# jondo2010/rust-ida

Hardware: AMD Instinct MI355X
Metric: Newton iters/sec (fp64), batched dense DAE N=512 B=4096 (higher is better)
Workload: dtype f64; 1 GPU; random linear dense index-1 DAE F=A y'+B y-c (SURVEY 8(d) config 3), N=512, B=4096 systems per GPU, rtol 1e-6 atol 1e-8, t=0..1 with 10 outputs, every system restarts on its own when it reaches t=1 (endless stream of integrations); n=512, batch_per_gpu=4096, total_batch=4096, lu_period=1, groups_per_gpu=4, mutually_concurrent_streams=4

## Files before the change

### rust-ida_amd/csrc/exp_switches.hpp

```cpp
#pragma once

#if !defined(IDAHIP_TIMING_BUILD) &&                                                                                   \
    (defined(IDAHIP_EXP_NOPRO) || defined(IDAHIP_EXP_NOUPD) || defined(IDAHIP_EXP_NOGATHER) || defined(IDAHIP_EXP_NODIAG) || \
     defined(IDAHIP_EXP_NOSWEEP) || defined(IDAHIP_STAMPS) || defined(IDAHIP_TRAIL_PIPE) || defined(IDAHIP_TRAIL_QUAD) ||   \
     defined(IDAHIP_WP_RING) || defined(IDAHIP_US_PAD) || defined(IDAHIP_SYS_UNR) || defined(IDAHIP_TRAIL_AHEAD) ||         \
     defined(IDAHIP_NT_SYS) || defined(IDAHIP_NT_SOLVE) || defined(IDAHIP_NT_FINALIZE) || defined(IDAHIP_NT_TRAIL))
#error "IDAHIP_EXP_* / IDAHIP_STAMPS / IDAHIP_TRAIL_* (IDAHIP_TRAIL_AHEAD: 0..3) / IDAHIP_WP_RING / IDAHIP_US_PAD / IDAHIP_SYS_UNR / IDAHIP_NT_* are timing-build switches: add -DIDAHIP_TIMING_BUILD (the library then reports itself as one and is not a product)"
#endif

namespace idahip {
namespace tb {

#ifdef IDAHIP_TIMING_BUILD
constexpr bool TIMING_BUILD = true;
#else
constexpr bool TIMING_BUILD = false;
#endif

#ifdef IDAHIP_EXP_NOPRO
constexpr bool NOPRO = true;
#else
constexpr bool NOPRO = false;
#endif
#ifdef IDAHIP_EXP_NOUPD
constexpr bool NOUPD = true;
#else
constexpr bool NOUPD = false;
#endif
#ifdef IDAHIP_EXP_NOGATHER
constexpr bool NOGATHER = true;
#else
constexpr bool NOGATHER = false;
#endif
#ifdef IDAHIP_EXP_NODIAG
constexpr bool NODIAG = true;
#else
constexpr bool NODIAG = false;
#endif
#ifdef IDAHIP_EXP_NOSWEEP
constexpr bool NOSWEEP = true;
#else
constexpr bool NOSWEEP = false;
#endif
#ifdef IDAHIP_STAMPS
constexpr int STAMPS = IDAHIP_STAMPS;
#else
constexpr int STAMPS = -1;
#endif
#ifdef IDAHIP_TRAIL_PIPE
constexpr bool TRAIL_PIPE = IDAHIP_TRAIL_PIPE != 0;
#else
constexpr bool TRAIL_PIPE = true;
#endif
#ifdef IDAHIP_TRAIL_QUAD
constexpr bool TRAIL_QUAD = IDAHIP_TRAIL_QUAD != 0;
#else
constexpr bool TRAIL_QUAD = true;
#endif
#ifdef IDAHIP_US_PAD
constexpr int US_PAD = IDAHIP_US_PAD;
#else
constexpr int US_PAD = 2;
#endif
#ifdef IDAHIP_TRAIL_AHEAD
constexpr int trail_ahead(int kk) { return IDAHIP_TRAIL_AHEAD; }
#else
constexpr int trail_ahead(int kk) { return kk < 32 ? 1 : 3; }
#endif
#ifdef IDAHIP_WP_RING
constexpr bool WP_DEEP_RING = IDAHIP_WP_RING != 0;
#else
constexpr bool WP_DEEP_RING = false;
#endif
#ifdef IDAHIP_SYS_UNR
constexpr int SYS_UNR = IDAHIP_SYS_UNR;
#else
constexpr int SYS_UNR = 16;
#endif

#ifdef IDAHIP_NT_SYS
constexpr bool NT_SYS = IDAHIP_NT_SYS != 0;
#else
constexpr bool NT_SYS = true;
#endif
#ifdef IDAHIP_NT_SOLVE
constexpr bool NT_SOLVE = IDAHIP_NT_SOLVE != 0;
#else
constexpr bool NT_SOLVE = true;
#endif
#ifdef IDAHIP_NT_FINALIZE
constexpr bool NT_FINALIZE = IDAHIP_NT_FINALIZE != 0;
#else
constexpr bool NT_FINALIZE = true;
#endif
#ifdef IDAHIP_NT_TRAIL
constexpr bool NT_TRAIL = IDAHIP_NT_TRAIL != 0;
#else
constexpr bool NT_TRAIL = false;
#endif

}
}
```

### rust-ida_amd/csrc/idahip.hip

```cpp
#include "common.hpp"
#include "lu_kernels.hpp"
#include "lu_driver.hpp"
#include "problem_kernels.hpp"
#include "solve_kernels.hpp"
#include "band_kernels.hpp"
#include "dq_kernels.hpp"
#include "vector_kernels.hpp"
#include "ic_kernels.hpp"
#include "tiny_ida.hpp"
#include "round_ida.hpp"

using namespace idahip;

namespace {

template <class T>
int dalloc(idahip_ctx* c, T** p, size_t count) {
    *p = nullptr;
    if (count == 0) return 0;
    IDAHIP_HIP(c, hipMalloc((void**)p, count * sizeof(T)));
    return 0;
}

int check_list(idahip_ctx* c, const int32_t* hIdx, int nsys) {
// ... 1819 lines not shown
        if (e == hipSuccess) e = hipStreamSynchronize(c->stream);
        if (e != hipSuccess) rc = fail(c, -100, "idahip_pow_batch: %s", hipGetErrorString(e));
    }
    if (dx) (void)hipFree(dx);
    if (dy) (void)hipFree(dy);
    if (dout) (void)hipFree(dout);
    return rc;
}

static int stepper_buffers(idahip_ctx* c, const idahip_tiny_call* call, bool outputs);

static FlowArgs flow_args(idahip_ctx* c, const idahip_tiny_call* call) {
    FlowArgs f;
    f.touts = c->tiny_touts; f.ntout = call->ntout; f.recycle = call->recycle; f.resume = call->resume;
    f.mxstep = call->mxstep; f.maxord = call->maxord; f.maxnef = call->maxnef; f.maxncf = call->maxncf;
    f.epcon = call->epcon; f.hmax_inv = call->hmax_inv; f.t0 = call->t0;
    f.start_round = call->start_round ? (const long long*)c->tiny_start : nullptr;
    f.acc = (unsigned long long*)c->tiny_acc;
    f.batch = c->batch;
    f.nrt = call->nroots;
    for (int i = 0; i < call->nroots && i < IDAHIP_MAX_ROOTS; ++i) {
        f.rt_comp[i] = call->root_comps[i];
        f.rt_thr[i] = call->root_thresholds[i];
    }
    return f;
}

int idahip_tiny_solve(idahip_ctx* c, void* hSys, size_t sys_bytes, const idahip_tiny_call* call, int64_t* hRoundsDone, uint64_t* hAcc,
                      double* hYout, double* hYPout) {
    DevGuard dev_guard__(c);
    if (!c) return -1;
    if (!hSys || !call || !hRoundsDone || !hAcc || !call->touts || call->ntout < 1) return fail(c, -2, "null argument");
    if (sys_bytes != sizeof(idactl::SysCore)) return fail(c, -2, "controller state of %zu bytes, this library expects %zu", sys_bytes, sizeof(idactl::SysCore));
    if (c->n != 3 || (c->kind != IDAHIP_ROBERTS && c->kind != IDAHIP_LORENZ63))
        return fail(c, -2, "the device-resident stepper takes the Roberts and Lorenz63 problems (n = 3)");
    if (c->jac_dq && !c->h_constr.empty()) return fail(c, -2, "difference-quotient Jacobians and constraints do not combine (DESIGN.md section 4g)");
    if (call->recycle && (!c->ic_y || !c->ic_yp)) return fail(c, -2, "recycle needs idahip_snapshot_initial");
    if (call->recycle && call->max_rounds < 1) return fail(c, -2, "recycle needs a round limit");
    const int batch = c->batch, n = c->n;
    int rc = stepper_buffers(c, call, hYout || hYPout);
    if (rc) return rc;
    const size_t ysz = (size_t)call->ntout * batch * n;
    IDAHIP_HIP(c, hipMemcpyAsync(c->tiny_sys, hSys, (size_t)batch * sizeof(idactl::SysCore), hipMemcpyHostToDevice, c->stream));
    IDAHIP_HIP(c, hipMemcpyAsync(c->tiny_touts, call->touts, sizeof(double) * call->ntout, hipMemcpyHostToDevice, c->stream));
    if (call->start_round)
        IDAHIP_HIP(c, hipMemcpyAsync(c->tiny_start, call->start_round, sizeof(int64_t) * batch, hipMemcpyHostToDevice, c->stream));
    IDAHIP_HIP(c, hipMemsetAsync(c->tiny_acc, 0, 2 * sizeof(uint64_t), c->stream));
    TinyIdaArgs a;
    a.sys = (idactl::SysCore*)c->tiny_sys;
    a.v = vec_state(c);
    a.savres = c->savres; a.lu = c->lu; a.piv = (long long*)c->piv; a.params = c->params; a.nparam = c->nparam;
    a.ic_y = c->ic_y; a.ic_yp = c->ic_yp;
    a.f = flow_args(c, call);
    a.roots = (idahip_root_state*)c->tiny_roots;
    a.jac_dq = c->jac_dq;
    a.max_rounds = call->max_rounds;
    a.round_base = call->round_base;
    a.yout = hYout ? c->tiny_yout : nullptr;
    a.ypout = hYPout ? c->tiny_ypout : nullptr;
    a.rounds_done = (long long*)c->tiny_rounds;
    {
        KTimer kt(c, IDAHIP_K_VECTOR, batch);
        int spw = 64;
        {
            const int simds = c->simds > 0 ? c->simds : 1024;
            while (spw > 1 && (long)(batch + spw / 2 - 1) / (spw / 2) <= simds / 4) spw >>= 1;
            if (const char* e = std::getenv("IDAHIP_TINY_SPW")) {
                const int v = (int)std::strtol(e, nullptr, 10);
                if (v == 1 || v == 2 || v == 4 || v == 8 || v == 16 || v == 32 || v == 64) spw = v;
            }
        }
        const size_t lds_state = (size_t)spw * sizeof(idactl::SysCore), lds_all = lds_state + (size_t)spw * sizeof(double) * tiny_lds_doubles(n);
        const bool roots = call->nroots > 0;
        const bool constr = !c->h_constr.empty();
        auto kern = c->kind == IDAHIP_ROBERTS ? (roots ? tiny_ida_kernel<IDAHIP_ROBERTS, true, false> : tiny_ida_kernel<IDAHIP_ROBERTS, false, false>)
                                              : (roots ? tiny_ida_kernel<IDAHIP_LORENZ63, true, false> : tiny_ida_kernel<IDAHIP_LORENZ63, false, false>);
        if (constr)
            kern = c->kind == IDAHIP_ROBERTS ? (roots ? tiny_ida_kernel<IDAHIP_ROBERTS, true, true> : tiny_ida_kernel<IDAHIP_ROBERTS, false, true>)
                                             : (roots ? tiny_ida_kernel<IDAHIP_LORENZ63, true, true> : tiny_ida_kernel<IDAHIP_LORENZ63, false, true>);
        const int lds_vec = hipFuncSetAttribute((const void*)kern, hipFuncAttributeMaxDynamicSharedMemorySize, (int)(64 * (sizeof(idactl::SysCore) + sizeof(double) * tiny_lds_doubles(n)))) == hipSuccess ? 1 : 0;
        if (!lds_vec) (void)hipGetLastError();
        const size_t shm = lds_vec ? lds_all : lds_state;
        hipLaunchKernelGGL(kern, dim3((batch + spw - 1) / spw), dim3(spw), shm, c->stream, a, lds_vec, constr ? (const double*)c->d_constr : (const double*)nullptr);
        if ((rc = post_launch(c, "tiny_ida"))) return rc;
    }
    IDAHIP_HIP(c, hipMemcpyAsync(hSys, c->tiny_sys, (size_t)batch * sizeof(idactl::SysCore), hipMemcpyDeviceToHost, c->stream));
    if (call->nroots > 0)
        IDAHIP_HIP(c, hipMemcpyAsync(call->root_states, c->tiny_roots, (size_t)batch * sizeof(idahip_root_state), hipMemcpyDeviceToHost, c->stream));
    IDAHIP_HIP(c, hipMemcpyAsync(hRoundsDone, c->tiny_rounds, sizeof(int64_t) * batch, hipMemcpyDeviceToHost, c->stream));
    IDAHIP_HIP(c, hipMemcpyAsync(hAcc, c->tiny_acc, 2 * sizeof(uint64_t), hipMemcpyDeviceToHost, c->stream));
    if (hYout) IDAHIP_HIP(c, hipMemcpyAsync(hYout, c->tiny_yout, sizeof(double) * ysz, hipMemcpyDeviceToHost, c->stream));
    if (hYPout) IDAHIP_HIP(c, hipMemcpyAsync(hYPout, c->tiny_ypout, sizeof(double) * ysz, hipMemcpyDeviceToHost, c->stream));
    IDAHIP_HIP(c, hipStreamSynchronize(c->stream));
    return 0;
}

static int stepper_buffers(idahip_ctx* c, const idahip_tiny_call* call, bool outputs) {
    const int batch = c->batch, n = c->n;
    int rc = 0;
    if (!c->tiny_sys) IDAHIP_HIP(c, hipMalloc(&c->tiny_sys, (size_t)batch * sizeof(idactl::SysCore)));
    if (!c->tiny_start) rc |= dalloc(c, &c->tiny_start, (size_t)batch);
    if (!c->tiny_rounds) rc |= dalloc(c, &c->tiny_rounds, (size_t)batch);
    if (!c->tiny_acc) rc |= dalloc(c, &c->tiny_acc, (size_t)2);
    if (rc) return rc;
    if (call->nroots < 0 || call->nroots > IDAHIP_MAX_ROOTS) return fail(c, -2, "the device steppers take at most %d root functions", IDAHIP_MAX_ROOTS);
    if (call->nroots > 0) {
        if (!call->root_comps || !call->root_thresholds || !call->root_states) return fail(c, -2, "root functions without their arrays");
        for (int i = 0; i < call->nroots; ++i)
            if (call->root_comps[i] < 0 || call->root_comps[i] >= n) return fail(c, -2, "root function %d watches component %d of %d", i, call->root_comps[i], n);
        if (call->recycle) return fail(c, -2, "root finding and idaens_stream's restarts do not combine");
        if (!c->tiny_roots) IDAHIP_HIP(c, hipMalloc(&c->tiny_roots, (size_t)batch * sizeof(idahip_root_state)));
        IDAHIP_HIP(c, hipMemcpyAsync(c->tiny_roots, call->root_states, (size_t)batch * sizeof(idahip_root_state), hipMemcpyHostToDevice, c->stream));
    }
    if (call->ntout > c->tiny_ntout_cap) {
        if (c->tiny_touts) (void)hipFree(c->tiny_touts);
        c->tiny_touts = nullptr;
        if ((rc = dalloc(c, &c->tiny_touts, (size_t)call->ntout))) return rc;
        c->tiny_ntout_cap = call->ntout;
    }
    if (outputs && call->ntout > c->tiny_yout_cap) {
        const size_t ysz = (size_t)call->ntout * batch * n;
        if (c->tiny_yout) (void)hipFree(c->tiny_yout);
        if (c->tiny_ypout) (void)hipFree(c->tiny_ypout);
        c->tiny_yout = c->tiny_ypout = nullptr;
        if ((rc = dalloc(c, &c->tiny_yout, ysz))) return rc;
        if ((rc = dalloc(c, &c->tiny_ypout, ysz))) return rc;
        c->tiny_yout_cap = call->ntout;
    }
    return 0;
}

int idahip_round_solve(idahip_ctx* c, void* hSys, size_t sys_bytes, const idahip_tiny_call* call, int64_t* hRoundsDone, uint64_t* hAcc,
                       double* hYout, double* hYPout, int64_t* rounds_run) {
    DevGuard dev_guard__(c);
    if (!c) return -1;
    if (!hSys || !call || !hRoundsDone || !hAcc || !rounds_run || !call->touts || call->ntout < 1) return fail(c, -2, "null argument");
    if (sys_bytes != sizeof(idactl::SysCore)) return fail(c, -2, "controller state of %zu bytes, this library expects %zu", sys_bytes, sizeof(idactl::SysCore));
    const bool lin = c->kind == IDAHIP_LINEAR_DENSE && c->n <= LU_BIG_MAX_N;
    const bool heat = c->kind == IDAHIP_HEAT1D && c->n <= LU_BIG_MAX_N;
    if (c->n <= TINY_N || !(lin || heat) || c->lu_variant < 4)
        return fail(c, -2, "the device-resident lock-step stepper takes linear dense and heat problems with %d < n <= %d (LU variant 4)", TINY_N, LU_BIG_MAX_N);
    if (!c->h_constr.empty()) return fail(c, -2, "the device lock-step stepper does not check constraints: the host stepper does (DESIGN.md section 4g)");
    if (call->recycle && (!c->ic_y || !c->ic_yp)) return fail(c, -2, "recycle needs idahip_snapshot_initial");
    if (call->recycle && call->max_rounds < 1) return fail(c, -2, "recycle needs a round limit");
    const int batch = c->batch, n = c->n;
    const long nn = (long)n * n;
    int rc = stepper_buffers(c, call, hYout || hYPout);
    if (rc) return rc;
    if (!c->rnd_i) rc |= dalloc(c, &c->rnd_i, (size_t)8 * batch + 8 + 2 * IDAHIP_K_COUNT);
    if (!c->rnd_d) rc |= dalloc(c, &c->rnd_d, (size_t)4 * batch);
    if (rc) return rc;
    if (!c->rnd_host) IDAHIP_HIP(c, hipHostMalloc((void**)&c->rnd_host, 4 * sizeof(int32_t)));
    const size_t ysz = (size_t)call->ntout * batch * n;
    IDAHIP_HIP(c, hipMemcpyAsync(c->tiny_sys, hSys, (size_t)batch * sizeof(idactl::SysCore), hipMemcpyHostToDevice, c->stream));
    IDAHIP_HIP(c, hipMemcpyAsync(c->tiny_touts, call->touts, sizeof(double) * call->ntout, hipMemcpyHostToDevice, c->stream));
    if (call->start_round)
        IDAHIP_HIP(c, hipMemcpyAsync(c->tiny_start, call->start_round, sizeof(int64_t) * batch, hipMemcpyHostToDevice, c->stream));
    IDAHIP_HIP(c, hipMemsetAsync(c->tiny_acc, 0, 2 * sizeof(uint64_t), c->stream));
    RoundArgs a;
    a.f = flow_args(c, call);
    a.sys = (idactl::SysCore*)c->tiny_sys;
    a.v = vec_state(c);
    a.ic_y = c->ic_y; a.ic_yp = c->ic_yp;
    a.yout = hYout ? c->tiny_yout : nullptr;
    a.ypout = hYPout ? c->tiny_ypout : nullptr;
    a.round_base = call->round_base;
    a.fused_jac = (c->kind == IDAHIP_LINEAR_DENSE && !c->jac_dq) ? 1 : 0;
    if (c->jac_dq && !c->dq_hh && (rc = dalloc(c, &c->dq_hh, (size_t)batch))) return rc;
    a.lu_period = c->lu_period;
    a.roots = (idahip_root_state*)c->tiny_roots;
    int* ib = c->rnd_i;
    a.stepping = ib; a.in_newton = ib + batch; a.skipP = ib + 2 * batch; a.skipL = ib + 3 * batch; a.skipI = ib + 4 * batch;
    a.skipS = ib + 5 * batch; a.ident = ib + 6 * batch; a.lu_list = ib + 7 * batch; a.lu_cnt = ib + 8 * batch; a.summary = ib + 8 * batch + 1; a.lu_wait = ib + 8 * batch + 3;
    a.stats = (unsigned long long*)(ib + 8 * batch + 4);
    if (((uintptr_t)a.stats & 7) != 0) a.stats = (unsigned long long*)(ib + 8 * batch + 5);
    IDAHIP_HIP(c, hipMemsetAsync(a.stats, 0, IDAHIP_K_COUNT * sizeof(unsigned long long), c->stream));
    a.lu_info = c->lu_info;
    a.tn = c->rnd_d; a.cj = c->rnd_d + batch; a.scale = c->rnd_d + 2 * batch; a.nrm_out = c->rnd_d + 3 * batch;
    a.rounds_done = (long long*)c->tiny_rounds;
    hipLaunchKernelGGL(round_init_kernel, dim3((batch + 255) / 256), dim3(256), 0, c->stream, a);
    IDAHIP_HIP(c, hipMemsetAsync(a.summary, 0, 2 * sizeof(int), c->stream));
    const size_t shm_wg = sizeof(double) * (4 * (size_t)n + 8);
    const size_t shm_it = 2 * sizeof(double) * n;
    SysArgs sa;
    fill_sys_args(c, sa, 1);
    sa.idx = a.ident; sa.tn = a.tn; sa.cj = a.cj;
    int64_t r = 0;
    for (;; ++r) {
        if (call->max_rounds > 0 && r >= call->max_rounds) break;
        a.round = r;
        a.first_round = r == 0;
        {
            KTimer kt(c, IDAHIP_K_VECTOR, 0);
            if (call->nroots > 0) hipLaunchKernelGGL(round_begin_kernel<true>, dim3(batch), dim3(WG_NT), shm_wg, c->stream, a);
            else hipLaunchKernelGGL(round_begin_kernel<false>, dim3(batch), dim3(WG_NT), shm_wg, c->stream, a);
            hipLaunchKernelGGL(round_lists_kernel, dim3(1), dim3(1024), 0, c->stream, a);
        }
        const bool lu_cnt_on_host = n > LU_MAX_N && !c->band;
        if (lu_cnt_on_host) {
            IDAHIP_HIP(c, hipMemcpyAsync(c->rnd_host + 2, a.lu_cnt, sizeof(int), hipMemcpyDeviceToHost, c->stream));
            IDAHIP_HIP(c, hipEventRecord(c->ev_cnt, c->stream));
        }
        {
            KTimer kt(c, IDAHIP_K_SYS, 0);
            sa.reset_ee = 1; sa.skip = a.skipP;
            if ((rc = launch_sys(c, sa, batch, nullptr))) return rc;
        }
        if (a.fused_jac) {
            KTimer kt(c, IDAHIP_K_SYS_JAC, 0);
            sa.skip = a.skipL;
            if ((rc = launch_sys(c, sa, batch, c->jw))) return rc;
        } else {
            {
                KTimer kt(c, IDAHIP_K_SYS, 0);
                sa.skip = a.skipL;
                if ((rc = launch_sys(c, sa, batch, nullptr))) return rc;
            }
            KTimer kt(c, IDAHIP_K_JAC, 0);
            if (c->jac_dq)
                hipLaunchKernelGGL(dq_round_prep_kernel, dim3((batch + 255) / 256), dim3(256), 0, c->stream, a.sys, (const int*)a.skipL, c->dq_hh,
                                   batch, dq_evals(c));
            if ((rc = launch_jac(c, c->jw, a.ident, a.cj, batch, nullptr, nullptr, nullptr, a.skipL, c->dq_hh))) return rc;
        }
        {
            int nlu = batch;
            const int* d_cnt = a.lu_cnt;
            if (lu_cnt_on_host) {
                IDAHIP_HIP(c, hipEventSynchronize(c->ev_cnt));
                nlu = c->rnd_host[2];
                d_cnt = nullptr;
                if (nlu < 0 || nlu > batch) return fail(c, -4, "list length %d outside 0..%d", nlu, batch);
            }
            KTimer kt(c, IDAHIP_K_LU, 0);
            if (c->band) rc = band_factor(c, c->bab, (long)c->ldab * n, c->piv, n, c->ml, c->mu, a.lu_list, nlu, d_cnt);
            else rc = lu_factor_batched(c, c->jw, nn, c->lu, nn, (long long*)c->piv, n, c->perm, a.lu_list, nlu, d_cnt);
            if (rc) return rc;
            if ((rc = post_launch(c, "lu"))) return rc;
        }
        hipLaunchKernelGGL(round_newton_ctl_kernel, dim3((batch + 255) / 256), dim3(256), 0, c->stream, a, 0);
        for (int m = 1; m <= idactl::MAXNLSIT; ++m) {
            {
                KTimer kt(c, IDAHIP_K_NEWTON_ITER, 0);
                if ((rc = launch_newton_iter(c, a.ident, a.scale, a.nrm_out, a.skipI, batch))) return rc;
            }
            hipLaunchKernelGGL(round_newton_ctl_kernel, dim3((batch + 255) / 256), dim3(256), 0, c->stream, a, m);
            if (m < idactl::MAXNLSIT) {
                KTimer kt(c, IDAHIP_K_SYS, 0);
                sa.reset_ee = 0; sa.skip = a.skipS;
                if ((rc = launch_sys(c, sa, batch, nullptr))) return rc;
            }
        }
        IDAHIP_HIP(c, hipMemsetAsync(a.summary, 0, sizeof(int), c->stream));
        {
            KTimer kt(c, IDAHIP_K_VECTOR, 0);
            if (call->nroots > 0) hipLaunchKernelGGL(round_end_kernel<true>, dim3(batch), dim3(WG_NT), shm_wg, c->stream, a);
            else hipLaunchKernelGGL(round_end_kernel<false>, dim3(batch), dim3(WG_NT), shm_wg, c->stream, a);
            if ((rc = post_launch(c, "round_end"))) return rc;
        }
        if (!call->recycle) {
            IDAHIP_HIP(c, hipMemcpyAsync(c->rnd_host, a.summary, 2 * sizeof(int), hipMemcpyDeviceToHost, c->stream));
            IDAHIP_HIP(c, hipStreamSynchronize(c->stream));
            if (c->rnd_host[0] == 0) {
                ++r;
                break;
            }
        }
    }
    (void)shm_it;
    *rounds_run = r;
    IDAHIP_HIP(c, hipMemcpyAsync(hSys, c->tiny_sys, (size_t)batch * sizeof(idactl::SysCore), hipMemcpyDeviceToHost, c->stream));
    if (call->nroots > 0)
        IDAHIP_HIP(c, hipMemcpyAsync(call->root_states, c->tiny_roots, (size_t)batch * sizeof(idahip_root_state), hipMemcpyDeviceToHost, c->stream));
    IDAHIP_HIP(c, hipMemcpyAsync(hRoundsDone, c->tiny_rounds, sizeof(int64_t) * batch, hipMemcpyDeviceToHost, c->stream));
    IDAHIP_HIP(c, hipMemcpyAsync(hAcc, c->tiny_acc, 2 * sizeof(uint64_t), hipMemcpyDeviceToHost, c->stream));
    if (hYout) IDAHIP_HIP(c, hipMemcpyAsync(hYout, c->tiny_yout, sizeof(double) * ysz, hipMemcpyDeviceToHost, c->stream));
    if (hYPout) IDAHIP_HIP(c, hipMemcpyAsync(hYPout, c->tiny_ypout, sizeof(double) * ysz, hipMemcpyDeviceToHost, c->stream));
    unsigned long long hstats[IDAHIP_K_COUNT];
    IDAHIP_HIP(c, hipMemcpyAsync(hstats, a.stats, sizeof hstats, hipMemcpyDeviceToHost, c->stream));
    IDAHIP_HIP(c, hipStreamSynchronize(c->stream));
    for (int k = 0; k < IDAHIP_K_COUNT; ++k) c->k_systems[k] += (int64_t)hstats[k];
    c->k_systems[IDAHIP_K_VECTOR] += 2 * r * (int64_t)batch;
    return 0;
}

int idahip_lu_variant(const idahip_ctx* c) { return c ? c->lu_variant : -1; }
int idahip_timing_build(void) { return tb::TIMING_BUILD ? 1 : 0; }
int idahip_set_lu_superpanel(idahip_ctx* c, int on) {
    if (!c) return -1;
    c->lu_superpanel = on != 0 ? 1 : 0;
    return 0;
}
int idahip_lu_superpanel(const idahip_ctx* c) { return c ? c->lu_superpanel : -1; }
int idahip_set_lu_period(idahip_ctx* c, int rounds) {
    if (!c || rounds < 1 || rounds > 64) return -1;
    c->lu_period = rounds;
    return 0;
}
int idahip_lu_period(const idahip_ctx* c) { return c ? c->lu_period : -1; }

int idahip_ls_type(const idahip_ctx* c) { return c ? IDAHIP_LS_DIRECT : -1; }
int idahip_ls_num_iters(const idahip_ctx* c) { return c ? 0 : -1; }
double idahip_ls_res_norm(const idahip_ctx* c) { (void)c; return 0.0; }

#ifdef IDAHIP_STAMPS
void* idahip_debug_stamps(idahip_ctx* c, size_t words) {
    if (!c) return nullptr;
    if (!c->dbg_stamps && hipMalloc((void**)&c->dbg_stamps, words * 8) != hipSuccess) return nullptr;
    (void)hipMemset(c->dbg_stamps, 0, words * 8);
    return c->dbg_stamps;
}
#endif

int idahip_set_lu_variant(idahip_ctx* c, int variant) {
    DevGuard dev_guard__(c);
    if (!c || variant < 3 || variant > 4) return -1;
    c->lu_variant = variant;
    return 0;
}

int idahip_timing_enable(idahip_ctx* c, int on) {
    DevGuard dev_guard__(c);
    if (!c) return -1;
    c->timing = on < 0 ? 0 : (on > 2 ? 2 : on);
    return 0;
}
int idahip_timing_get(idahip_ctx* c, idahip_kclass k, double* ms, int64_t* launches, int64_t* systems) {
    DevGuard dev_guard__(c);
    if (!c || k < 0 || k >= IDAHIP_K_COUNT) return -1;
    if (ms) *ms = c->k_ms[k];
    if (launches) *launches = c->k_launches[k];
    if (systems) *systems = c->k_systems[k];
    return 0;
}
int idahip_timing_reset(idahip_ctx* c) {
    DevGuard dev_guard__(c);
    if (!c) return -1;
    for (int k = 0; k < IDAHIP_K_COUNT; ++k) {
        c->k_ms[k] = 0.0;
        c->k_launches[k] = 0;
        c->k_systems[k] = 0;
    }
    return 0;
}

}
```

### rust-ida_amd/csrc/lu_driver.hpp

```cpp
#pragma once
#include "lu_kernels.hpp"
#include "lu_wavepanel.hpp"
#include "lu_superpanel.hpp"

namespace idahip {

inline int lu_factor_batched(idahip_ctx* c, double* work, long wstride, double* out, long ostride, long long* piv, long pstride,
                             int* perm, const int* d_idx, int nsys, const int* d_cnt = nullptr) {
    const int n = c->n;
    if (nsys == 0) return 0;
    if (n <= TINY_N) {
        hipLaunchKernelGGL(tiny_getrf_kernel, dim3((nsys + 63) / 64), dim3(64), 0, c->stream, work, wstride, d_idx, nsys, n, piv,
                           pstride, perm, c->lu_info);
        return 0;
    }
    if (n > LU_BIG_MAX_N) return fail(c, -3, "blocked LU supports n <= %d in this build (n = %d)", LU_BIG_MAX_N, n);
    if (d_cnt && c->lu_variant < 4) return fail(c, -3, "a device-side list length needs LU variant 4");
    LuWs w;
    w.mats = work; w.mstride = wstride; w.idx = d_idx; w.cnt = d_cnt; w.n = n;
    w.pos = c->lu_pos; w.live = c->lu_live; w.prow = c->lu_prow; w.piv = piv; w.pstride = pstride; w.info = c->lu_info; w.redo = c->lu_redo; w.nzb = c->lu_nzb; w.bz = c->lu_bz;
    w.zmap = (out == c->lu) ? c->lu_zmap : nullptr;
    w.dirty = (out == c->lu) ? c->lu_dirty : nullptr;
    w.jwzero = (w.dirty && work == c->jw && c->lu_superpanel && n > LU_MAX_N) ? c->lu_jwzero : nullptr;
    if (!w.jwzero && c->lu_jwzero && (work == c->jw || out == c->jw))
        (void)hipMemsetAsync(c->lu_jwzero, 0, (size_t)c->batch * sizeof(int), c->stream);
    w.l11 = c->lu_l11; w.stamps = c->dbg_stamps; w.out = out; w.ostride = ostride; w.l11ld = 64;
    hipLaunchKernelGGL(lu_init_kernel, dim3(nsys), dim3(256), 0, c->stream, w);
    const int nsys8 = ((nsys + 7) / 8) * 8;
    constexpr int NB = LU_NB;
    auto panel2 = [&](int k0, int lbase) {
        const int threads = (((n - k0 + 1) / 2 + 63) / 64) * 64;
        hipLaunchKernelGGL((lu_panel2_kernel<NB, 512, 2>), dim3(nsys), dim3(threads), 0, c->stream, w, k0, lbase);
    };
    for (int k0 = 0; k0 < n; k0 += 64) {
        if (n - k0 > LU_MAX_N) {
            KTimer kt(c, IDAHIP_K_LU_PANEL, nsys);
            const int cend = (k0 + 64 < n) ? k0 + 64 : n;
            if (c->lu_superpanel) {
                if (n - k0 > LU_WIDE_ROWS) {
                    const int threads = (((n - k0 + 7) / 8 + 63) / 64) * 64;
                    hipLaunchKernelGGL((lu_superpanel_kernel<8, 512, 2>), dim3(nsys), dim3(threads), 0, c->stream, w, k0);
                } else {
                    const int threads = (((n - k0 + 3) / 4 + 63) / 64) * 64;
                    hipLaunchKernelGGL((lu_superpanel_kernel<4, 512, 2>), dim3(nsys), dim3(threads), 0, c->stream, w, k0);
                }
            } else {
            auto narrow_split = [&](int kk, int nbs) {
                const int ntiles = (n - kk - nbs + 63) / 64;
                return ntiles >= 32 ? 8 : ntiles >= 16 ? 4 : ntiles >= 8 ? 2 : 1;
            };
            if (n - k0 > LU_WIDE_ROWS) {
                constexpr int NBS = 8;
                const int threads = (((n - k0 + 7) / 8 + 63) / 64) * 64;
                for (int lb = 0; lb < 64 && k0 + lb < n; lb += NBS) {
                    hipLaunchKernelGGL((lu_panelr_kernel<NBS, 8, 512, 2>), dim3(nsys), dim3(threads), 0, c->stream, w, k0 + lb, lb);
                    if (k0 + lb + NBS < cend) {
                        const int nsplit = narrow_split(k0 + lb, NBS);
                        hipLaunchKernelGGL((lu_trail_kernel<NBS, LU_BIG_MAX_N, 4>), dim3(nsys8 * nsplit), dim3(256), 0, c->stream, w, k0 + lb, nsys, 1,
                                           cend, lb * 65, nsplit);
                    }
                }
            } else {
                constexpr int NBS = 16;
                const int threads = (((n - k0 + 3) / 4 + 63) / 64) * 64;
                for (int lb = 0; lb < 64 && k0 + lb < n; lb += NBS) {
                    hipLaunchKernelGGL((lu_panelr_kernel<NBS, 4, 512, 2>), dim3(nsys), dim3(threads), 0, c->stream, w, k0 + lb, lb);
                    if (k0 + lb + NBS < cend) {
                        const int nsplit = narrow_split(k0 + lb, NBS);
                        hipLaunchKernelGGL((lu_trail_kernel<NBS, LU_BIG_MAX_N, 4>), dim3(nsys8 * nsplit), dim3(256), 0, c->stream, w, k0 + lb, nsys, 1,
                                           cend, lb * 65, nsplit);
                    }
                }
            }
            }
        } else if (c->lu_superpanel && c->lu_variant >= 4 && n > LU_MAX_N && n - k0 >= 64) {
            KTimer kt(c, IDAHIP_K_LU_PANEL, nsys);
            const int threads = (((n - k0 + 1) / 2 + 63) / 64) * 64;
            hipLaunchKernelGGL((lu_superpanel_kernel<2, 512, 2>), dim3(nsys), dim3(threads), 0, c->stream, w, k0);
        } else if (c->lu_variant >= 4 && n - k0 <= WP_MAX_ROWS) {
            KTimer kt(c, IDAHIP_K_LU_PANEL, nsys);
            const int ns = (n - k0 + 63) / 64;
#define IDAHIP_WP_LAUNCH(NSV) \
    hipLaunchKernelGGL((lu_wavepanel_kernel<false, NSV>), dim3(nsys), dim3(64), 0, c->stream, w, k0)
#define IDAHIP_WP_SWITCH()                                                                                    \
    switch (ns) {                                                                                              \
        case 1: IDAHIP_WP_LAUNCH(1); break;                                                                 \
        case 2: IDAHIP_WP_LAUNCH(2); break;                                                                 \
        case 3: IDAHIP_WP_LAUNCH(3); break;                                                                 \
        case 4: IDAHIP_WP_LAUNCH(4); break;                                                                 \
        case 5: IDAHIP_WP_LAUNCH(5); break;                                                                 \
        case 6: IDAHIP_WP_LAUNCH(6); break;                                                                 \
        case 7: IDAHIP_WP_LAUNCH(7); break;                                                                 \
        default: IDAHIP_WP_LAUNCH(8); break;                                                                \
    }
            IDAHIP_WP_SWITCH()
            hipLaunchKernelGGL((lu_wavepanel_kernel<true, 0>), dim3(nsys), dim3(64), 0, c->stream, w, k0);
#undef IDAHIP_WP_SWITCH
#undef IDAHIP_WP_LAUNCH
        } else {
            KTimer kt(c, IDAHIP_K_LU_PANEL, nsys);
            panel2(k0, 0);
            if (n - k0 > NB) {
                const int cend = (k0 + 64 < n) ? k0 + 64 : n;
                hipLaunchKernelGGL((lu_trail_kernel<NB, LU_MAX_N, 2>), dim3(nsys8), dim3(256), 0, c->stream, w, k0, nsys, 1, cend, 0, 1);
                panel2(k0 + NB, NB);
            }
        }
        const int ntrail = n - k0 - 64;
        if (ntrail > 0) {
            KTimer kt(c, IDAHIP_K_LU_TRAIL, nsys);
            const int ncb = (ntrail + 63) / 64;
            if (n > LU_MAX_N) {
                const int nstrips = (ntrail + 15) / 16;
                int nsplit = nstrips >= 64 ? 8 : nstrips >= 32 ? 4 : nstrips >= 16 ? 2 : 1;
                while (!d_cnt && nsplit > 1 && nsys * nsplit > 512) nsplit >>= 1;
                const int nbs = nsplit > 1 ? std::min(ncb, LU_SPLIT_BLOCKS) : 0;
                hipLaunchKernelGGL(lu_u12_zero_kernel, dim3(nsys8 * ncb), dim3(256), 0, c->stream, w, k0, nsys, ncb);
                hipLaunchKernelGGL(lu_trail64w_kernel<LU_BIG_MAX_N>, dim3(nsys8 * (ncb + (nsplit - 1) * nbs)), dim3(256), 0, c->stream, w, k0, nsys, ncb, nsplit);
            } else
                hipLaunchKernelGGL(lu_trail64w_kernel<LU_MAX_N>, dim3(nsys8 * ncb), dim3(256), 0, c->stream, w, k0, nsys, ncb, 1);
        }
    }
    {
        KTimer kt(c, IDAHIP_K_LU_FINALIZE, nsys);
        hipLaunchKernelGGL(lu_finalize_kernel, dim3(nsys, (n + 31) / 32), dim3(256), 0, c->stream, w, out, ostride, perm, 32, NB,
                           n > LU_MAX_N ? (c->lu_superpanel ? 64 : 8) : 0,
                           c->lu_variant >= 4 ? ((c->lu_superpanel && n > LU_MAX_N) ? LU_MAX_N : WP_MAX_ROWS) : 0);
    }
    return 0;
}

}
```

### rust-ida_amd/csrc/lu_wavepanel.hpp

```cpp
#pragma once
#include <type_traits>

#include "lu_kernels.hpp"

namespace idahip {

constexpr int WP_MAX_ROWS = 512;
constexpr int WP_RING(int ns) { return !tb::WP_DEEP_RING ? 2 : (ns >= 1 && ns <= 2) ? 8 : (ns >= 3 && ns <= 7) ? 4 : 2; }

template <bool SLOWK, int NS>
__global__ __launch_bounds__(64, SLOWK ? 1 : (NS > 0 && NS <= 3 ? 4 : 2)) void lu_wavepanel_kernel(LuWs w, const int k0) {
    constexpr int BIG = 1 << 20;
    if (w.cnt && (int)blockIdx.x >= *w.cnt) return;
    const int b = w.idx[blockIdx.x];
    if (w.info[b] != 0) return;
    const int n = w.n;
    double* __restrict__ A = w.mats + (long)b * w.mstride;
    int* __restrict__ pos = w.pos + (long)b * n;
    int* __restrict__ live = w.live + (long)b * n;
    int* __restrict__ prow = w.prow + (long)b * n;
    long long* __restrict__ piv = w.piv + (long)b * w.pstride;
    double* __restrict__ l11 = w.l11 + (long)b * L11_STRIDE;

    const __amdgpu_buffer_rsrc_t rsrc = __builtin_amdgcn_make_buffer_rsrc(A, 0, n * n * 8, 0x00020000);
    const int m = n - k0;
    const int wsp = m < 64 ? m : 64;
    const int lane = threadIdx.x;
    const int nslots = NS > 0 ? NS : (m + 63) >> 6;
    constexpr int NSC = NS > 0 ? NS : 8;

    __shared__ int ptab[64];

    int rowid[8], rpos[8], pstep[8];
    unsigned roff[8];
    static_for<0, NSC>([&](auto st) {
        constexpr int S = decltype(st)::value;
        const int li = S * 64 + lane;
        const bool has = li < m;
        rowid[S] = has ? live[li] : 0;
        rpos[S] = has ? pos[rowid[S]] : 0x7fffffff;
        pstep[S] = has ? BIG : -1;
        roff[S] = (unsigned)rowid[S] * 8u;
    });

    auto load_block = [&](double (&x)[8][8], const int b8, const int wb) {
        static_for<0, NSC>([&](auto st) {
            constexpr int S = decltype(st)::value;
            if (S < nslots) {
                const double* __restrict__ src = A + (long)(k0 + b8) * n + rowid[S];
#pragma unroll
                for (int j = 0; j < 8; ++j) x[S][j] = (j < wb) ? src[(long)j * n] : 0.0;
            } else {
#pragma unroll
                for (int j = 0; j < 8; ++j) x[S][j] = 0.0;
            }
        });
    };
    auto store_block = [&](const double (&x)[8][8], const int b8, const int wb) {
        static_for<0, NSC>([&](auto st) {
            constexpr int S = decltype(st)::value;
            if (S < nslots && pstep[S] >= 0) {
                double* __restrict__ dst = A + (long)(k0 + b8) * n + rowid[S];
#pragma unroll
                for (int j = 0; j < 8; ++j)
                    if (j < wb) dst[(long)j * n] = x[S][j];
            }
        });
    };

    auto process = [&](auto slow_tag, double (&x)[8][8], const int b8, const int wb) -> int {
        constexpr bool SLOW = decltype(slow_tag)::value;
        if (b8 > 0) {
            auto load_l = [&](double (&l)[8], const int k) {
                const int coloff = (k0 + k) * n * 8;
                static_for<0, NSC>([&](auto st) {
                    constexpr int S = decltype(st)::value;
                    l[S] = buf_load_f64(rsrc, roff[S], coloff);
                });
            };
            auto apply = [&](const double (&l)[8], const int k, const int ow) {
                const int pl = __builtin_amdgcn_readfirstlane(ow) & 63, ps = __builtin_amdgcn_readfirstlane(ow) >> 6;
                double uk[8];
                switch (ps) {
#define IDAHIP_WP_CASE(SV)                                                                     \
    case SV:                                                                                   \
        if constexpr (SV < NSC) {                                                              \
            _Pragma("unroll") for (int j = 0; j < 8; ++j) uk[j] = readlane_f64(x[SV][j], pl); \
        }                                                                                      \
        break;
                    IDAHIP_WP_CASE(1)
                    IDAHIP_WP_CASE(2)
                    IDAHIP_WP_CASE(3)
                    IDAHIP_WP_CASE(4)
                    IDAHIP_WP_CASE(5)
                    IDAHIP_WP_CASE(6)
                    IDAHIP_WP_CASE(7)
                    default:
                        IDAHIP_WP_CASE(0)
#undef IDAHIP_WP_CASE
                }
                double ukv[8];
                if (SLOW) {
#pragma unroll
                    for (int j = 0; j < 8; ++j) ukv[j] = opaque_vgpr(uk[j]);
                }
                static_for<0, NSC>([&](auto st) {
                    constexpr int S = decltype(st)::value;
                    if (S < nslots) {
                        if (pstep[S] > k) {
#pragma unroll
                            for (int j = 0; j < 8; ++j) {
                                if (SLOW) {
                                    const double tn = upd(x[S][j], ukv[j], l[S]);
                                    x[S][j] = (ukv[j] == 0.0) ? x[S][j] : tn;
                                } else {
                                    x[S][j] = upd(x[S][j], uk[j], l[S]);
                                }
                            }
                        }
                    }
                });
            };
            __builtin_amdgcn_s_waitcnt(0x0F70);
            constexpr int D = WP_RING(NS);
            double l[D][8];
            int ow[D];
            static_for<0, D>([&](auto dt) {
                constexpr int d = decltype(dt)::value;
                load_l(l[d], d);
                ow[d] = ptab[d];
            });
#pragma unroll 1
            for (int k = 0; k < b8; k += D) {
                static_for<0, D>([&](auto dt) {
                    constexpr int d = decltype(dt)::value;
                    apply(l[d], k + d, ow[d]);
                    const int kn = (k + d + D < b8) ? k + d + D : b8 - 1;
                    load_l(l[d], kn);
                    ow[d] = ptab[kn];
                });
            }
        }
        bool special = false;
        int status = 0, failcol = 0;
        static_for<0, 8>([&](auto kt) {
            constexpr int kk = decltype(kt)::value;
            const bool active = !SLOW || (status == 0 && kk < wb);
            const int kstep = b8 + kk, kc = k0 + kstep;
            unsigned kh[8], kl[8];
            static_for<0, NSC>([&](auto st) {
                constexpr int S = decltype(st)::value;
                const double v = x[S][kk];
                unsigned h = (unsigned)__double2hiint(v) | 0x80000000u, l = (unsigned)__double2loint(v);
                if (SLOW) {
                    if (v != v) {
                        h = (rpos[S] == kc) ? 0xfff00000u : 0u;
                        l = 0u;
                    }
                }
                kh[S] = (pstep[S] == BIG) ? h : 0u;
                kl[S] = l;
            });
            unsigned lm = kh[0];
#pragma unroll
            for (int s = 1; s < NSC; ++s) lm = kh[s] > lm ? kh[s] : lm;
            const unsigned mh = wave_max_u32<false>(lm);
            if (!SLOW) special = special || mh >= 0xfff00000u;
            int cnt = 0, slot = 0;
#pragma unroll
            for (int s = 0; s < NSC; ++s) {
                const bool e = kh[s] == mh;
                cnt += e ? 1 : 0;
                slot = e ? s : slot;
            }
            const unsigned long long bal = __ballot(cnt > 0);
            int pl = (int)__ffsll((unsigned long long)bal) - 1;
            int ps;
            if (__popcll(bal) == 1 && __builtin_amdgcn_readlane(cnt, pl) == 1) {
                ps = __builtin_amdgcn_readlane(slot, pl);
            } else {
                unsigned bl = 0u;
                int bp_ = 0x7fffffff, bs = 0;
#pragma unroll
                for (int s = 0; s < NSC; ++s) {
                    const bool e = kh[s] == mh;
                    const bool better = e && (kl[s] > bl || (kl[s] == bl && rpos[s] < bp_) || bp_ == 0x7fffffff);
                    bl = better ? kl[s] : bl;
                    bp_ = better ? rpos[s] : bp_;
                    bs = better ? s : bs;
                }
                const bool e1 = bp_ != 0x7fffffff;
                const unsigned ml = wave_max_u32<false>(e1 ? bl : 0u);
                const bool top = e1 && bl == ml;
                const int pm = wave_min_i32f<false>(top ? bp_ : 0x7fffffff);
                const unsigned long long b2 = __ballot(top && bp_ == pm);
                pl = (int)__ffsll((unsigned long long)b2) - 1;
                ps = __builtin_amdgcn_readlane(bs, pl);
            }
            double u[8];
            int bp = 0, pr = 0;
            switch (ps) {
#define IDAHIP_WP_CASE(SV)                                                                             \
    case SV:                                                                                           \
        if constexpr (SV < NSC) {                                                                      \
            _Pragma("unroll") for (int j = kk; j < 8; ++j) u[j] = readlane_f64(x[SV][j], pl);         \
            bp = __builtin_amdgcn_readlane(rpos[SV], pl);                                              \
            pr = __builtin_amdgcn_readlane(rowid[SV], pl);                                             \
        }                                                                                              \
        break;
                IDAHIP_WP_CASE(1)
                IDAHIP_WP_CASE(2)
                IDAHIP_WP_CASE(3)
                IDAHIP_WP_CASE(4)
                IDAHIP_WP_CASE(5)
                IDAHIP_WP_CASE(6)
                IDAHIP_WP_CASE(7)
                default:
                    IDAHIP_WP_CASE(0)
#undef IDAHIP_WP_CASE
            }
            bool go = active;
            if (active && u[kk] == 0.0) {
                status = 1;
                failcol = kc + 1;
                go = !SLOW;
            }
            const double recip = 1.0 / u[kk];
            if (go) {
                if (lane == 0) {
                    piv[kc] = (long long)bp;
                    prow[kc] = pr;
                    ptab[kstep] = pl | (ps << 6);
                }
                __builtin_amdgcn_fence(__ATOMIC_RELEASE, "wavefront");
                __builtin_amdgcn_wave_barrier();
                static_for<0, NSC>([&](auto st) {
                    constexpr int S = decltype(st)::value;
                    if (pstep[S] == BIG && rpos[S] == kc) rpos[S] = bp;
                    if (lane == pl && ps == S) {
                        pstep[S] = kstep;
                        rpos[S] = kc;
                    }
                });
            }
            double uv[8];
            if (SLOW) {
#pragma unroll
                for (int j = kk + 1; j < 8; ++j) uv[j] = opaque_vgpr(u[j]);
            }
            static_for<0, NSC>([&](auto st) {
                constexpr int S = decltype(st)::value;
                if (S < nslots) {
                    if (pstep[S] == BIG && go) {
                        const double l = x[S][kk] * recip;
                        x[S][kk] = l;
#pragma unroll
                        for (int j = kk + 1; j < 8; ++j) {
                            if (SLOW) {
                                const double tn = upd(x[S][j], uv[j], l);
                                x[S][j] = (uv[j] == 0.0) ? x[S][j] : tn;
                            } else {
                                x[S][j] = upd(x[S][j], u[j], l);
                            }
                        }
                    }
                }
            });
        });
        if (!SLOW) {
            bool z = false;
            static_for<0, NSC>([&](auto st) {
                constexpr int S = decltype(st)::value;
                bool zz = false;
#pragma unroll
                for (int j = 0; j < 8; ++j) zz = zz || (x[S][j] == 0.0 && j < wb);
                z = z || (zz && pstep[S] >= 0 && pstep[S] != BIG);
            });
            if (special || status != 0 || __ballot(z) != 0ull) return 2;
        }
        if (status == 1 && lane == 0) w.info[b] = failcol;
        return status;
    };

    int bstart = 0;
    if (SLOWK) {
        const int rd = w.redo[b];
        if (rd == 0) return;
        bstart = (rd - 1) * 8;
        for (int k = 0; k < bstart; ++k) {
            const int kc = k0 + k;
            const int bp = (int)piv[kc], pr = prow[kc];
            static_for<0, NSC>([&](auto st) {
                constexpr int S = decltype(st)::value;
                if (pstep[S] == BIG && rpos[S] == kc) rpos[S] = bp;
                const bool mine = pstep[S] >= 0 && rowid[S] == pr;
                if (mine) {
                    pstep[S] = k;
                    rpos[S] = kc;
                }
                const unsigned long long bm = __ballot(mine);
                if (bm != 0ull && lane == 0) ptab[k] = ((int)__ffsll((unsigned long long)bm) - 1) | (S << 6);
            });
            __builtin_amdgcn_fence(__ATOMIC_RELEASE, "wavefront");
            __builtin_amdgcn_wave_barrier();
        }
        if (lane == 0) w.redo[b] = 0;
    }
    for (int b8 = bstart; b8 < wsp; b8 += 8) {
        const int wb = (wsp - b8) < 8 ? (wsp - b8) : 8;
        double x[8][8];
        int st;
        if (SLOWK) {
            load_block(x, b8, wb);
            st = process(std::true_type{}, x, b8, wb);
        } else {
            if (wb != 8) {
                st = 2;
            } else {
                load_block(x, b8, 8);
                st = process(std::false_type{}, x, b8, 8);
            }
            if (st == 2) {
                if (lane == 0) w.redo[b] = 1 + (b8 >> 3);
                return;
            }
        }
        if (st != 0) return;
        store_block(x, b8, wb);
    }

    __syncthreads();
    static_for<0, NSC>([&](auto st) {
        constexpr int S = decltype(st)::value;
        if (pstep[S] >= 0) pos[rowid[S]] = rpos[S];
    });
    if (lane < wsp) {
        const double* __restrict__ src = A + (long)k0 * n + prow[k0 + lane];
        for (int j0 = 0; j0 < lane; j0 += 8) {
            double v[8];
#pragma unroll
            for (int u = 0; u < 8; ++u) v[u] = (j0 + u < lane) ? src[(long)(j0 + u) * n] : 0.0;
#pragma unroll
            for (int u = 0; u < 8; ++u)
                if (j0 + u < lane) l11[(j0 + u) * 64 + lane] = v[u];
        }
    }
    int base = 0;
    static_for<0, NSC>([&](auto st) {
        constexpr int S = decltype(st)::value;
        const bool al = pstep[S] == BIG;
        const unsigned long long bal = __ballot(al);
        if (al) live[base + __popcll(bal & ((1ull << lane) - 1ull))] = rowid[S];
        base += __popcll(bal);
    });
}

}
```

Before: 361,600 Newton iters/s.

## Allow packing several systems per workgroup in wavepanel LU kernel

Templates the wavepanel LU panel kernel on a waves-per-workgroup count W, so each 64-lane wave handles its own system and its own slice of shared ptab, with launch grids shrunk accordingly. The workgroup-wide __syncthreads is replaced by a wavefront-scope fence, waitcnt and wave barrier, since only intra-wave ordering is needed. Default pack factors are 1, so the launch shape is unchanged unless timing-build switches are set. An optional hardware-ID stamping probe is also added.

```diff
diff --git a/rust-ida_amd/csrc/exp_switches.hpp b/rust-ida_amd/csrc/exp_switches.hpp
--- a/rust-ida_amd/csrc/exp_switches.hpp
+++ b/rust-ida_amd/csrc/exp_switches.hpp
@@ -4,8 +4,9 @@
     (defined(IDAHIP_EXP_NOPRO) || defined(IDAHIP_EXP_NOUPD) || defined(IDAHIP_EXP_NOGATHER) || defined(IDAHIP_EXP_NODIAG) || \
      defined(IDAHIP_EXP_NOSWEEP) || defined(IDAHIP_STAMPS) || defined(IDAHIP_TRAIL_PIPE) || defined(IDAHIP_TRAIL_QUAD) ||   \
      defined(IDAHIP_WP_RING) || defined(IDAHIP_US_PAD) || defined(IDAHIP_SYS_UNR) || defined(IDAHIP_TRAIL_AHEAD) ||         \
-     defined(IDAHIP_NT_SYS) || defined(IDAHIP_NT_SOLVE) || defined(IDAHIP_NT_FINALIZE) || defined(IDAHIP_NT_TRAIL))
-#error "IDAHIP_EXP_* / IDAHIP_STAMPS / IDAHIP_TRAIL_* (IDAHIP_TRAIL_AHEAD: 0..3) / IDAHIP_WP_RING / IDAHIP_US_PAD / IDAHIP_SYS_UNR / IDAHIP_NT_* are timing-build switches: add -DIDAHIP_TIMING_BUILD (the library then reports itself as one and is not a product)"
+     defined(IDAHIP_NT_SYS) || defined(IDAHIP_NT_SOLVE) || defined(IDAHIP_NT_FINALIZE) || defined(IDAHIP_NT_TRAIL) ||      \
+     defined(IDAHIP_WP_PACK) || defined(IDAHIP_WP_PACK_LO) || defined(IDAHIP_WP_PACK_SLOW) || defined(IDAHIP_WP_HWID))
+#error "IDAHIP_EXP_* / IDAHIP_STAMPS / IDAHIP_TRAIL_* (IDAHIP_TRAIL_AHEAD: 0..3) / IDAHIP_WP_RING / IDAHIP_WP_PACK* / IDAHIP_WP_HWID / IDAHIP_US_PAD / IDAHIP_SYS_UNR / IDAHIP_NT_* are timing-build switches: add -DIDAHIP_TIMING_BUILD (the library then reports itself as one and is not a product)"
 #endif
 
 namespace idahip {
@@ -72,6 +73,30 @@
 #else
 constexpr bool WP_DEEP_RING = false;
 #endif
+#ifdef IDAHIP_WP_PACK
+constexpr int WP_PACK = IDAHIP_WP_PACK;
+#else
+constexpr int WP_PACK = 1;
+#endif
+#ifdef IDAHIP_WP_PACK_LO
+constexpr int WP_PACK_LO = IDAHIP_WP_PACK_LO;
+#else
+constexpr int WP_PACK_LO = 1;
+#endif
+#ifdef IDAHIP_WP_PACK_SLOW
+constexpr int WP_PACK_SLOW = IDAHIP_WP_PACK_SLOW;
+#else
+constexpr int WP_PACK_SLOW = 1;
+#endif
+constexpr int wp_pack(bool slowk, int ns) { return slowk ? WP_PACK_SLOW : (ns >= 1 && ns <= 3) ? WP_PACK_LO : WP_PACK; }
+static_assert((WP_PACK == 1 || WP_PACK == 2 || WP_PACK == 4 || WP_PACK == 8) && (WP_PACK_LO == 1 || WP_PACK_LO == 2 || WP_PACK_LO == 4 || WP_PACK_LO == 8) &&
+                  (WP_PACK_SLOW == 1 || WP_PACK_SLOW == 2 || WP_PACK_SLOW == 4),
+              "waves per workgroup of lu_wavepanel_kernel: 1, 2, 4 or 8 (SLOW: at most 4)");
+#ifdef IDAHIP_WP_HWID
+constexpr bool WP_HWID = true;
+#else
+constexpr bool WP_HWID = false;
+#endif
 #ifdef IDAHIP_SYS_UNR
 constexpr int SYS_UNR = IDAHIP_SYS_UNR;
 #else
diff --git a/rust-ida_amd/csrc/idahip.hip b/rust-ida_amd/csrc/idahip.hip
--- a/rust-ida_amd/csrc/idahip.hip
+++ b/rust-ida_amd/csrc/idahip.hip
@@ -2145,7 +2145,7 @@
 int idahip_ls_num_iters(const idahip_ctx* c) { return c ? 0 : -1; }
 double idahip_ls_res_norm(const idahip_ctx* c) { (void)c; return 0.0; }
 
-#ifdef IDAHIP_STAMPS
+#if defined(IDAHIP_STAMPS) || defined(IDAHIP_WP_HWID)
 void* idahip_debug_stamps(idahip_ctx* c, size_t words) {
     if (!c) return nullptr;
     if (!c->dbg_stamps && hipMalloc((void**)&c->dbg_stamps, words * 8) != hipSuccess) return nullptr;
diff --git a/rust-ida_amd/csrc/lu_driver.hpp b/rust-ida_amd/csrc/lu_driver.hpp
--- a/rust-ida_amd/csrc/lu_driver.hpp
+++ b/rust-ida_amd/csrc/lu_driver.hpp
@@ -80,8 +80,10 @@
         } else if (c->lu_variant >= 4 && n - k0 <= WP_MAX_ROWS) {
             KTimer kt(c, IDAHIP_K_LU_PANEL, nsys);
             const int ns = (n - k0 + 63) / 64;
-#define IDAHIP_WP_LAUNCH(NSV) \
-    hipLaunchKernelGGL((lu_wavepanel_kernel<false, NSV>), dim3(nsys), dim3(64), 0, c->stream, w, k0)
+#define IDAHIP_WP_LAUNCH(NSV)                                                                                              \
+    hipLaunchKernelGGL((lu_wavepanel_kernel<false, NSV, tb::wp_pack(false, NSV)>),                                         \
+                       dim3((nsys + tb::wp_pack(false, NSV) - 1) / tb::wp_pack(false, NSV)), dim3(64 * tb::wp_pack(false, NSV)), 0, \
+                       c->stream, w, k0, nsys)
 #define IDAHIP_WP_SWITCH()                                                                                    \
     switch (ns) {                                                                                              \
         case 1: IDAHIP_WP_LAUNCH(1); break;                                                                 \
@@ -94,7 +96,10 @@
         default: IDAHIP_WP_LAUNCH(8); break;                                                                \
     }
             IDAHIP_WP_SWITCH()
-            hipLaunchKernelGGL((lu_wavepanel_kernel<true, 0>), dim3(nsys), dim3(64), 0, c->stream, w, k0);
+            {
+                constexpr int WS = tb::wp_pack(true, 0);
+                hipLaunchKernelGGL((lu_wavepanel_kernel<true, 0, WS>), dim3((nsys + WS - 1) / WS), dim3(64 * WS), 0, c->stream, w, k0, nsys);
+            }
 #undef IDAHIP_WP_SWITCH
 #undef IDAHIP_WP_LAUNCH
         } else {
diff --git a/rust-ida_amd/csrc/lu_wavepanel.hpp b/rust-ida_amd/csrc/lu_wavepanel.hpp
--- a/rust-ida_amd/csrc/lu_wavepanel.hpp
+++ b/rust-ida_amd/csrc/lu_wavepanel.hpp
@@ -8,11 +8,14 @@
 constexpr int WP_MAX_ROWS = 512;
 constexpr int WP_RING(int ns) { return !tb::WP_DEEP_RING ? 2 : (ns >= 1 && ns <= 2) ? 8 : (ns >= 3 && ns <= 7) ? 4 : 2; }
 
-template <bool SLOWK, int NS>
-__global__ __launch_bounds__(64, SLOWK ? 1 : (NS > 0 && NS <= 3 ? 4 : 2)) void lu_wavepanel_kernel(LuWs w, const int k0) {
+template <bool SLOWK, int NS, int W>
+__global__ __launch_bounds__(64 * W, SLOWK ? 1 : (NS > 0 && NS <= 3 ? 4 : 2)) void lu_wavepanel_kernel(LuWs w, const int k0, const int nsys) {
     constexpr int BIG = 1 << 20;
-    if (w.cnt && (int)blockIdx.x >= *w.cnt) return;
-    const int b = w.idx[blockIdx.x];
+    const int wave = W > 1 ? __builtin_amdgcn_readfirstlane((int)threadIdx.x >> 6) : 0;
+    const int li0 = (int)blockIdx.x * W + wave;
+    if (W > 1 && li0 >= nsys) return;
+    if (w.cnt && li0 >= *w.cnt) return;
+    const int b = w.idx[li0];
     if (w.info[b] != 0) return;
     const int n = w.n;
     double* __restrict__ A = w.mats + (long)b * w.mstride;
@@ -25,11 +28,20 @@
     const __amdgpu_buffer_rsrc_t rsrc = __builtin_amdgcn_make_buffer_rsrc(A, 0, n * n * 8, 0x00020000);
     const int m = n - k0;
     const int wsp = m < 64 ? m : 64;
-    const int lane = threadIdx.x;
+    const int lane = W > 1 ? (int)threadIdx.x & 63 : (int)threadIdx.x;
     const int nslots = NS > 0 ? NS : (m + 63) >> 6;
     constexpr int NSC = NS > 0 ? NS : 8;
 
-    __shared__ int ptab[64];
+    __shared__ int ptab_all[W][64];
+    int* const ptab = ptab_all[wave];
+    if constexpr (tb::WP_HWID && !SLOWK) {
+        if (w.stamps && lane == 0) {
+            unsigned hw, xcc;
+            asm volatile("s_getreg_b32 %0, hwreg(HW_REG_HW_ID)" : "=s"(hw));
+            asm volatile("s_getreg_b32 %0, hwreg(HW_REG_XCC_ID)" : "=s"(xcc));
+            w.stamps[(size_t)(k0 >> 6) * nsys + li0] = (1ull << 63) | ((unsigned long long)(xcc & 15u) << 32) | hw;
+        }
+    }
 
     int rowid[8], rpos[8], pstep[8];
     unsigned roff[8];
@@ -329,7 +341,9 @@
         store_block(x, b8, wb);
     }
 
-    __syncthreads();
+    __builtin_amdgcn_fence(__ATOMIC_RELEASE, "wavefront");
+    __builtin_amdgcn_s_waitcnt(0x0F70);
+    __builtin_amdgcn_wave_barrier();
     static_for<0, NSC>([&](auto st) {
         constexpr int S = decltype(st)::value;
         if (pstep[S] >= 0) pos[rowid[S]] = rpos[S];
```

Result: no change. 362,200 Newton iters/s (median of 5 runs) (+0.2%).
